# yamatokataoka/reinforcement-learning-replications

Measured on NVIDIA H100. Metric: ppo_update_transitions_per_sec, higher is better.
Workload: dtype f32

## Files before the change

reinforcement-learning-replications_b200/csrc/mlp_tc3.cu:

```cuda
#include <cuda_fp16.h>

#include <cmath>

#include "common.cuh"
#include "policy_head.cuh"
#include "tc2_common.cuh"
#include "tc_common.cuh"
#include "tc3.cuh"

namespace b200rl {

constexpr int T3_ROWS = 128;
constexpr int T3_CHAIN_WARPS = 8;
constexpr int T3_THREADS = T3_CHAIN_WARPS * 32 + 256;
constexpr int T3_WARPS = T3_THREADS / 32;

constexpr uint32_t S3_XB = 0;
constexpr uint32_t S3_H1 = 2 * T2_ACT;
constexpr uint32_t S3_H2 = S3_H1 + 2 * T2_ACT;
constexpr uint32_t S3_DZ2 = S3_H2 + 2 * T2_ACT;
constexpr uint32_t S3_DZ1 = S3_DZ2 + 2 * T2_ACT;
constexpr uint32_t T3_W1T = 32 * 128, T3_W2 = 64 * 128, T3_W3 = 16 * 128;
constexpr uint32_t S3_DO = S3_DZ1 + 2 * T2_ACT;
constexpr uint32_t S3_W = S3_DO + T2_ACT;
constexpr uint32_t S3_WNET = 2 * T3_W1T + 2 * T3_W2 + 2 * T3_W3;
constexpr uint32_t S3_OPERANDS_END = S3_W + S3_WNET;
constexpr uint32_t S3_BIAS = S3_OPERANDS_END;
constexpr uint32_t S3_DIST = S3_BIAS + 2 * 640;
constexpr uint32_t S3_SCALE = S3_DIST + 256;
constexpr uint32_t S3_XS = S3_SCALE + 128;
constexpr uint32_t S3_RED = S3_XS + 256;
constexpr uint32_t S3_BARS = S3_RED + 4 * 8 * T3_WARPS;
constexpr uint32_t S3_TOTAL = S3_BARS + 128;
constexpr uint32_t T3_SMEM_BYTES = S3_TOTAL + 1024;
static_assert(T3_SMEM_BYTES <= 227 * 1024, "mlp_tc3 shared memory");
constexpr uint32_t S3_END_DB3 = 0;
constexpr uint32_t S3_END_SC = 1024;

constexpr uint32_t ACC_GRAD_NET = 176;
constexpr uint32_t ACC_DB3 = 2 * ACC_GRAD_NET;
static_assert(ACC_DB3 + 4 * 16 <= ACC_COLS, "mlp_tc3 accumulator columns");
constexpr uint32_t ACC_DW2 = 0, ACC_DB2 = 64, ACC_DW1 = 80, ACC_DW3 = 144;

__device__ __forceinline__ uint32_t grad_acc_off(uint32_t pcol, int n, int row, int col) {
  const int rr = row & 63;
  const int t = 32 * (rr >> 4) + 4 * (rr & 7) + ((col >> 1) & 3);
  const int e = 2 * ((rr >> 3) & 1) + (col & 1);
  return pcol * ACC_LANES + (uint32_t)((row >> 6) * 64 * n + 4 * (128 * (col >> 3) + t) + e);
}

#ifdef B200RL_TC3_TIMING
__device__ unsigned long long g_tc3_t[64];
#endif

enum { C3_G = 0, C3_U1, C3_U2, C3_U3, C3_UH2, C3_UH1, C3_W1, C3_W2, C3_W3, C3_OW3, C3_OW2, C3_OW1, C3_OB, C3_N };

__device__ __forceinline__ void mbar_arrive_expect_tx(uint32_t bar, uint32_t bytes) {
  asm volatile("mbarrier.arrive.expect_tx.shared::cta.b64 _, [%0], %1;" ::"r"(bar), "r"(bytes) : "memory");
}
__device__ __forceinline__ void bulk_copy_g2s(uint32_t dst_smem, const void* src, uint32_t bytes, uint32_t bar) {
  asm volatile("cp.async.bulk.shared::cluster.global.mbarrier::complete_tx::bytes [%0], [%1], %2, [%3];" ::"r"(dst_smem),
               "l"(src), "r"(bytes), "r"(bar)
               : "memory");
}

__global__ void __launch_bounds__(128) pack_obs_kernel(const float* __restrict__ obs, long long n_rows, int n_in,
                                                       const float* __restrict__ absmax, uint8_t* __restrict__ ximg,
                                                       float* __restrict__ xscale, float* __restrict__ bad_flag) {
  __shared__ float s_xs[32];
  const int r = threadIdx.x;
  bool bad = false;
  if (r < 32) {
    const int e = r < n_in ? fit_exp(__ldg(absmax + r), bad) : 0;
    s_xs[r] = pow2i(e);
    if (blockIdx.x == 0) {
      xscale[r] = pow2i(e);
      xscale[32 + r] = pow2i(-e);
    }
  }
  __syncthreads();
  const long long tiles = (n_rows + T3_ROWS - 1) / T3_ROWS;
  for (long long t = blockIdx.x; t < tiles; t += gridDim.x) {
    const long long row = t * T3_ROWS + r;
    float x[32];
#pragma unroll
    for (int c = 0; c < 32; ++c) x[c] = 0.f;
    if (row < n_rows) {
      const float* src = obs + row * n_in;
      float rmax = 0.f, probe = 0.f;
#pragma unroll
      for (int c = 0; c < 31; ++c)
        if (c < n_in) {
          x[c] = __ldg(src + c) * s_xs[c];
          rmax = fmaxf(rmax, fabsf(x[c]));
          probe += x[c];
        }
      if (!(rmax <= T2_RANGE) || probe != probe) bad = true;
      if (rmax > 0.f && rmax < 0.03125f) bad = true;
      x[31] = 1.0f;
    }
    uint4 h[4], l[4];
#pragma unroll
    for (int j = 0; j < 4; ++j) {
      split2h(x[8 * j + 0], x[8 * j + 1], h[j].x, l[j].x);
      split2h(x[8 * j + 2], x[8 * j + 3], h[j].y, l[j].y);
      split2h(x[8 * j + 4], x[8 * j + 5], h[j].z, l[j].z);
      split2h(x[8 * j + 6], x[8 * j + 7], h[j].w, l[j].w);
    }
    uint8_t* dst = ximg + (size_t)t * T2_ACT + (size_t)r * 128;
#pragma unroll
    for (int j = 0; j < 4; ++j) {
      *reinterpret_cast<uint4*>(dst + ((j ^ (r & 7)) << 4)) = h[j];
      *reinterpret_cast<uint4*>(dst + (((4 + j) ^ (r & 7)) << 4)) = l[j];
    }
  }
  if (bad) *bad_flag = 1.0f;
}

template <int N, int TA, int TB, int TERMS, int KSTEPS>
__device__ __forceinline__ void wg_mma(float (&d)[N / 2], const uint32_t (&alo)[TERMS], const uint32_t (&blo)[TERMS],
                                       uint32_t a_hi, uint32_t b_hi, uint32_t a_k, uint32_t b_k, uint32_t accumulate) {
  wgmma_fence();
#pragma unroll
  for (int s = 0; s < TERMS; ++s)
#pragma unroll
    for (int k = 0; k < KSTEPS; ++k)
      wgmma_run<N, TA, TB>(d, ((uint64_t)a_hi << 32) | (alo[s] + (uint32_t)k * a_k),
                           ((uint64_t)b_hi << 32) | (blo[s] + (uint32_t)k * b_k), s == 0 && k == 0 ? accumulate : 1u);
  wgmma_commit();
  wgmma_wait_all();
}
template <int N, int TB, int KSTEPS>
__device__ __forceinline__ void chain_mma(float (&d)[N / 2], const Op2 a, const Op2 b) {
  const uint32_t alo[3] = {a.lo, a.lo + a.split_step, a.lo}, blo[3] = {b.lo + b.split_step, b.lo, b.lo};
#pragma unroll
  for (int i = 0; i < N / 2; ++i) d[i] = 0.f;
  wg_mma<N, K_MAJOR, TB, 3, KSTEPS>(d, alo, blo, a.hi, b.hi, a.k_step, b.k_step, 0u);
}
__device__ __forceinline__ float* grad_frag(float* acc_cta, uint32_t pcol) {
  const int t = (int)(threadIdx.x & 127u);
  return acc_cta + grad_acc_off(pcol, 0, 16 * (t >> 5) + ((t & 31) >> 2), 2 * (t & 3));
}
template <int N, int KSTEPS, int TERMS>
__device__ __forceinline__ void grad_products(float (&d)[N / 2], uint32_t a_lo, const Op2 a, const Op2 b, bool first) {
  uint32_t b_lo = b.lo;
  asm volatile("" : "+r"(a_lo), "+r"(b_lo));
#pragma unroll
  for (int s = 0; s < TERMS; ++s)
#pragma unroll
    for (int k = 0; k < KSTEPS; ++k)
      wgmma_run<N, MN_MAJOR, MN_MAJOR>(d, ((uint64_t)a.hi << 32) | (a_lo + (uint32_t)k * a.k_step),
                                       ((uint64_t)b.hi << 32) | (b_lo + (s + 1 < TERMS ? b.split_step : 0u) +
                                                                 (uint32_t)k * b.k_step),
                                       s == 0 && k == 0 ? (first ? 0u : 1u) : 1u);
}
template <int N>
__device__ __forceinline__ void grad_store(float* acc_cta, uint32_t pcol, int h, const float (&d)[N / 2]) {
  float* const frag = grad_frag(acc_cta, pcol) + 64 * N * h;
#pragma unroll
  for (int j = 0; j < N / 8; ++j)
    *reinterpret_cast<float4*>(frag + 512 * j) = make_float4(d[4 * j], d[4 * j + 1], d[4 * j + 2], d[4 * j + 3]);
}

__global__ void __launch_bounds__(T3_THREADS, 1) mlp_tc3_kernel(const Tc3Args p) {
  extern __shared__ uint8_t smem_raw[];
  const bool two = p.run_policy != 0 && p.run_value != 0;
  const int G = two ? (int)(gridDim.x >> 1) : (int)gridDim.x;
  const int c = two ? (int)blockIdx.x / G : (p.run_policy != 0 ? 0 : 1);
  const int slot = (int)blockIdx.x - c * (two ? G : 0);
  const bool run_p = p.run_policy != 0 && (p.stop_flag == nullptr || *p.stop_flag == 0);
  const bool run_v = p.run_value != 0;
  if (!(c == 0 ? run_p : run_v)) return;
  if (*p.x_bad != 0.f) return;
  const int tid = threadIdx.x, lane = tid & 31;
  float* const acc = p.acc_mem + (size_t)slot * ACC_CTA_FLOATS;
  const int warp = __shfl_sync(0xffffffffu, tid >> 5, 0);
  const uint32_t raw = smem_u32(smem_raw);
  const uint32_t base = (raw + 1023u) & ~1023u;
  uint8_t* sm = smem_raw + (base - raw);
  float* s_bias = reinterpret_cast<float*>(sm + S3_BIAS);
  float* s_dist = reinterpret_cast<float*>(sm + S3_DIST);
  float* s_scale = reinterpret_cast<float*>(sm + S3_SCALE);
  float* s_xs = reinterpret_cast<float*>(sm + S3_XS);
  float* s_red = reinterpret_cast<float*>(sm + S3_RED);
  int* s_bad = reinterpret_cast<int*>(sm + S3_BARS + 120);
  const uint32_t bars = base + S3_BARS;
  const int n_in = p.n_in;
  bool bad = false;
#ifdef B200RL_TC3_TIMING
  unsigned long long tacc[64];
  for (int i = 0; i < 64; ++i) tacc[i] = 0;
  const long long t_kernel0 = clock64();
#endif

  for (uint32_t i = S3_W / 16 + tid; i < S3_OPERANDS_END / 16; i += T3_THREADS) reinterpret_cast<uint4*>(sm)[i] = make_uint4(0, 0, 0, 0);
  if (tid == 0) *s_bad = 0;
  if (tid < 64) s_xs[tid] = __ldg(p.xscale + tid);
  float* s_par = reinterpret_cast<float*>(sm + S3_H1);
  static_assert(S3_W - S3_H1 >= 4 * (2 * 6000 + 64), "parameter staging area");
#pragma unroll 1
  for (int net = 0; net < 2; ++net) {
    const float* par = p.params[net];
    float* dst = s_par + (net == 0 ? 0 : p.P[0]);
#pragma unroll 8
    for (int i = tid; i < p.P[net]; i += T3_THREADS) dst[i] = (*(par + i));
  }
  __syncthreads();
#pragma unroll 1
  for (int net = 0; net < 2; ++net) {
    const Tc3Net& nn = p.net[net];
    const float* par = s_par + (net == 0 ? 0 : p.P[0]);
    float m1 = 0.f, m2 = 0.f, m3 = 0.f;
    for (int idx = tid; idx < nn.h1 * n_in; idx += T3_THREADS) {
      const float w = (*(par + nn.w_off[0] + idx)) * s_xs[32 + idx % n_in];
      m1 = fmaxf(m1, fabsf(w));
      if (w != w) bad = true;
    }
    for (int idx = tid; idx < nn.h2 * nn.h1; idx += T3_THREADS) {
      const float w = (*(par + nn.w_off[1] + idx));
      m2 = fmaxf(m2, fabsf(w));
      if (w != w) bad = true;
    }
    for (int idx = tid; idx < nn.n_out * nn.h2; idx += T3_THREADS) {
      const float w = (*(par + nn.w_off[2] + idx));
      m3 = fmaxf(m3, fabsf(w));
      if (w != w) bad = true;
    }
#pragma unroll
    for (int o = 16; o > 0; o >>= 1) {
      m1 = fmaxf(m1, __shfl_xor_sync(0xffffffffu, m1, o));
      m2 = fmaxf(m2, __shfl_xor_sync(0xffffffffu, m2, o));
      m3 = fmaxf(m3, __shfl_xor_sync(0xffffffffu, m3, o));
    }
    if (lane == 0) {
      s_red[warp * 8 + 4 * net + 0] = m1;
      s_red[warp * 8 + 4 * net + 1] = m2;
      s_red[warp * 8 + 4 * net + 2] = m3;
    }
  }
  __syncthreads();
  if (bad) *s_bad = 1;
  bad = false;
  if (tid < 2) {
    const int net = tid;
    const Tc3Net& nn = p.net[net];
    float m1 = 0.f, m2 = 0.f, m3 = 0.f;
    for (int w = 0; w < T3_WARPS; ++w) {
      m1 = fmaxf(m1, s_red[w * 8 + 4 * net + 0]);
      m2 = fmaxf(m2, s_red[w * 8 + 4 * net + 1]);
      m3 = fmaxf(m3, s_red[w * 8 + 4 * net + 2]);
    }
    bool b0 = false;
    const int ew1 = fit_exp(m1, b0), ew2 = fit_exp(m2, b0), ew3 = fit_exp(m3, b0);
    float typ;
    if (net == 1) {
      const float tm = __ldg(p.target_absmax);
      typ = (tm > 0.f && tm < INFINITY) ? 0.25f * tm : 1.f;
    } else if (p.dist == B200RL_DIST_GAUSSIAN) {
      float smin = INFINITY;
      for (int a = 0; a < nn.n_out; ++a) smin = fminf(smin, expf(__ldg(p.log_std + a)));
      typ = (smin > 0.f && smin < INFINITY) ? 1.f / smin : 1.f;
    } else {
      typ = 0.5f;
    }
    int eg = 3 + ilogbf(p.n_glob_f) - ilogbf(typ);
    eg = eg < -100 ? -100 : (eg > 100 ? 100 : eg);
    float* sc = s_scale + 16 * net;
    sc[C3_G] = pow2i(eg);
    sc[C3_U1] = pow2i(-ew1);
    sc[C3_U2] = pow2i(-(T2_H_EXP + ew2));
    sc[C3_U3] = pow2i(-(T2_H_EXP + ew3));
    sc[C3_UH2] = pow2i(-ew3);
    sc[C3_UH1] = pow2i(-ew2);
    sc[C3_W1] = pow2i(ew1);
    sc[C3_W2] = pow2i(ew2);
    sc[C3_W3] = pow2i(ew3);
    sc[C3_OW3] = pow2i(-(T2_H_EXP + eg));
    sc[C3_OW2] = pow2i(-(T2_H_EXP + eg));
    sc[C3_OW1] = pow2i(-eg);
    sc[C3_OB] = pow2i(-eg);
    if (b0) *s_bad = 1;
  }
  __syncthreads();
#pragma unroll 1
  for (int net = 0; net < 2; ++net) {
    const Tc3Net& nn = p.net[net];
    const float* par = s_par + (net == 0 ? 0 : p.P[0]);
    const uint32_t wb = S3_W;
    auto put = [&](uint32_t buf, uint32_t stride, int r, int c, float x) {
      const __half hb = __float2half_rn(x);
      const __half lb = __float2half_rn(x - __half2float(hb));
      const uint32_t off = buf + (uint32_t)r * 128u + ((uint32_t)((c >> 3) ^ (r & 7)) << 4) + ((uint32_t)(c & 7) << 1);
      *reinterpret_cast<__half*>(sm + off) = hb;
      *reinterpret_cast<__half*>(sm + off + stride) = lb;
    };
    const float* sc = s_scale + 16 * net;
    const float sw1 = sc[C3_W1], sw2 = sc[C3_W2], sw3 = sc[C3_W3];
    if (net == c) {
      for (int idx = tid; idx < nn.h1 * n_in; idx += T3_THREADS)
        put(wb, T3_W1T, idx % n_in, idx / n_in, ((*(par + nn.w_off[0] + idx)) * s_xs[32 + idx % n_in]) * sw1);
      for (int idx = tid; idx < nn.h2 * nn.h1; idx += T3_THREADS)
        put(wb + 2 * T3_W1T, T3_W2, idx / nn.h1, idx % nn.h1, (*(par + nn.w_off[1] + idx)) * sw2);
      for (int idx = tid; idx < nn.n_out * nn.h2; idx += T3_THREADS)
        put(wb + 2 * T3_W1T + 2 * T3_W2, T3_W3, idx / nn.h2, idx % nn.h2, (*(par + nn.w_off[2] + idx)) * sw3);
    }
    float* bb = s_bias + 160 * net;
    for (int i = tid; i < 64; i += T3_THREADS) {
      bb[i] = i < nn.h1 ? (*(par + nn.b_off[0] + i)) : 0.f;
      bb[64 + i] = i < nn.h2 ? (*(par + nn.b_off[1] + i)) : 0.f;
      if (!(fabsf(bb[i]) < INFINITY) || !(fabsf(bb[64 + i]) < INFINITY)) bad = true;
    }
    for (int i = tid; i < 16; i += T3_THREADS) {
      bb[128 + i] = i < nn.n_out ? (*(par + nn.b_off[2] + i)) : 0.f;
      if (!(fabsf(bb[128 + i]) < INFINITY)) bad = true;
    }
  }
  if (p.dist == B200RL_DIST_GAUSSIAN)
    for (int a = tid; a < p.net[0].n_out; a += T3_THREADS) {
      const NormalConsts nc = normal_consts(p.log_std, a);
      s_dist[a] = nc.var;
      s_dist[16 + a] = nc.log_scale;
      s_dist[32 + a] = nc.inv_2var;
      s_dist[48 + a] = nc.inv_var;
    }
  if (bad) *s_bad = 1;
  bad = false;
  if (tid == 0) {
    mbar_init(bars + 0, 1);
    mbar_init(bars + 8, 1);
    for (int i = 0; i < 3; ++i) {
      mbar_init(bars + 16 + 8 * i, 2);
      mbar_init(bars + 40 + 8 * i, 2);
    }
    fence_mbar_init();
  }
  fence_proxy_async_smem();
  __syncthreads();

  const long long num_tiles = (p.n_rows + T3_ROWS - 1) / T3_ROWS;
  const int cta_tiles = (int)((num_tiles - slot + G - 1) / G);

  constexpr int K = K_MAJOR, MN = MN_MAJOR;
  const uint32_t ub = base;
  auto bar_ready = [&](int s) { return bars + 16u + 8u * (uint32_t)(s - 3); };
  auto bar_done = [&](int s) { return bars + 40u + 8u * (uint32_t)(s - 3); };
  double sc[5] = {0, 0, 0, 0, 0};
  int rows_done = 0;
#ifdef B200RL_TC3_TIMING
  long long t_loop0 = 0, t_loop_end = 0;
#endif

  if (warp >= T3_CHAIN_WARPS) {
    const Op2 X_M = op2_mnmajor(ub + S3_XB, T2_ACT, 64);
    const Op2 X_M16 = op2_mnmajor(ub + S3_XB + 32, T2_ACT, 64);
    const Op2 DO_M = op2_at(op2_mnmajor(ub + S3_DO, T2_ACT, 32), c * 64);
    const Op2 H1_M = op2_mnmajor(ub + S3_H1, T2_ACT, T2_ACT), H2_M = op2_mnmajor(ub + S3_H2, T2_ACT, T2_ACT);
    const Op2 DZ2_M = op2_mnmajor(ub + S3_DZ2, T2_ACT, T2_ACT), DZ1_M = op2_mnmajor(ub + S3_DZ1, T2_ACT, T2_ACT);
    const int g = (warp - T3_CHAIN_WARPS) >> 2;
    const bool producer = g == 0;
    const uint32_t ah = (uint32_t)g * (T2_ACT >> 4);
    const uint32_t gcol = c * ACC_GRAD_NET;
    float w3[16], w2[32], b2[8], w1[32];
    auto load_x = [&](int k) {
      const uint32_t b = (uint32_t)(k & 1);
      const long long tile = slot + (long long)k * G;
      uint32_t e;
      asm volatile("{\n\t.reg .pred q;\n\telect.sync _|q, 0xffffffff;\n\tselp.u32 %0, 1, 0, q;\n\t}" : "=r"(e));
      if (e && (warp & 3) == 0) {
        mbar_arrive_expect_tx(bars + 8 * b, T2_ACT);
        bulk_copy_g2s(ub + S3_XB + b * T2_ACT, p.ximg + (size_t)tile * T2_ACT, T2_ACT, bars + 8 * b);
      }
      __syncwarp();
    };
    auto release = [&](int stage) {
      wgmma_commit();
      wgmma_wait_all();
      asm volatile("bar.sync %0, 128;" ::"r"(8 + g) : "memory");
      if ((tid & 127) == 0) mbar_arrive(bar_done(stage));
    };
    if (producer && cta_tiles > 0) load_x(0);
#pragma unroll 1
    for (int k = 0; k < cta_tiles; ++k) {
      const uint32_t xo = (uint32_t)(k & 1) * T2_ACT;
      const bool first = k == 0;
      if (producer && k + 1 < cta_tiles) {
        if (k > 0) mbar_wait(bar_done(5), (uint32_t)((k - 1) & 1));
        load_x(k + 1);
      }
#ifdef B200RL_TC3_TIMING
      long long it0 = clock64(), it1;
#define TC3_GSPLIT(s)                                                   \
  it1 = clock64();                                                      \
  tacc[40 + 3 * g + (s) - 3] += (unsigned long long)(it1 - it0);
#define TC3_GEND(s)                                                     \
  it0 = clock64();                                                      \
  tacc[46 + 3 * g + (s) - 3] += (unsigned long long)(it0 - it1);
#else
#define TC3_GSPLIT(s)
#define TC3_GEND(s)
#endif
      mbar_wait(bar_ready(3), (uint32_t)(k & 1));
      TC3_GSPLIT(3)
      wgmma_fence();
      grad_products<32, 8, 1>(w3, H2_M.lo + ah, H2_M, DO_M, first);
      release(3);
      TC3_GEND(3)
      mbar_wait(bar_ready(4), (uint32_t)(k & 1));
      TC3_GSPLIT(4)
      wgmma_fence();
      grad_products<64, 8, 2>(w2, DZ2_M.lo + ah, DZ2_M, H1_M, first);
      grad_products<16, 8, 1>(b2, DZ2_M.lo + ah, DZ2_M, op2_at(X_M16, xo), first);
      release(4);
      TC3_GEND(4)
      mbar_wait(bar_ready(5), (uint32_t)(k & 1));
      TC3_GSPLIT(5)
      wgmma_fence();
      grad_products<64, 8, 1>(w1, DZ1_M.lo + ah, DZ1_M, op2_at(X_M, xo), first);
      release(5);
      TC3_GEND(5)
#undef TC3_GSPLIT
#undef TC3_GEND
    }
    if (cta_tiles > 0) {
      grad_store<32>(acc, gcol + ACC_DW3, g, w3);
      grad_store<64>(acc, gcol + ACC_DW2, g, w2);
      grad_store<16>(acc, gcol + ACC_DB2, g, b2);
      grad_store<64>(acc, gcol + ACC_DW1, g, w1);
    }
#ifdef B200RL_TC3_TIMING
    if ((tid & 127) == 0 && blockIdx.x == 0) {
      for (int s = 0; s < 3; ++s) {
        g_tc3_t[40 + 3 * g + s] = tacc[40 + 3 * g + s];
        g_tc3_t[46 + 3 * g + s] = tacc[46 + 3 * g + s];
      }
      if (producer) g_tc3_t[52] = (unsigned long long)cta_tiles;
    }
#endif
  } else {
    const int wg = warp >> 2;
    const int quad = lane >> 2, q = lane & 3;
    const int r0 = 64 * wg + 16 * (warp & 3) + quad;
    const uint32_t rows = (uint32_t)wg * (64u * 128u);
    const Op2 X_K = op2_at(op2_kmajor(ub + S3_XB, 64), rows);
    const Op2 DO_K = op2_at(op2_kmajor(ub + S3_DO, 32), rows + c * 64);
    const Op2 H1_K = op2_at(op2_kmajor(ub + S3_H1, T2_ACT), rows), H2_K = op2_at(op2_kmajor(ub + S3_H2, T2_ACT), rows);
    const Op2 DZ2_K = op2_at(op2_kmajor(ub + S3_DZ2, T2_ACT), rows);
    const Op2 W1T_M = op2_mnmajor(ub + S3_W, 32 * 128, T3_W1T);
    const Op2 W2_K = op2_kmajor(ub + S3_W + 2 * T3_W1T, T3_W2), W2_M = op2_mnmajor(ub + S3_W + 2 * T3_W1T, 64 * 128, T3_W2);
    const Op2 W3_K = op2_kmajor(ub + S3_W + 2 * T3_W1T + 2 * T3_W2, T3_W3),
              W3_M = op2_mnmajor(ub + S3_W + 2 * T3_W1T + 2 * T3_W2, 16 * 128, T3_W3);
    const float* scl = s_scale + 16 * c;
    const float* bias = s_bias + 160 * c;
    const float sH = pow2i(T2_H_EXP), hh = pow2i(-2 * T2_H_EXP);
    const int A_out = p.net[0].n_out;

    auto frag_off = [&](uint32_t buf, int j, int r) -> uint32_t {
      return buf + (uint32_t)(r0 + 8 * r) * 128u + ((uint32_t)(j ^ quad) << 4) + 4u * (uint32_t)q;
    };
    auto store_pairs = [&](uint32_t buf, const float (&x)[32]) {
#pragma unroll
      for (int j = 0; j < 8; ++j)
#pragma unroll
        for (int r = 0; r < 2; ++r) {
          uint32_t h, l;
          split2h(x[4 * j + 2 * r], x[4 * j + 2 * r + 1], h, l);
          const uint32_t off = frag_off(buf, j, r);
          *reinterpret_cast<uint32_t*>(sm + off) = h;
          *reinterpret_cast<uint32_t*>(sm + off + T2_ACT) = l;
        }
    };
    auto act = [&](float (&z)[32], float unscale, const float* bs) {
#pragma unroll
      for (int g = 0; g < 2; ++g) {
        float t[16];
#pragma unroll
        for (int i = 0; i < 16; ++i) {
          const int e = 16 * g + i;
          t[i] = fmaf(z[e], unscale, bs[8 * (e >> 2) + 2 * q + (e & 1)]);
        }
        tanh16_scaled(t, sH);
#pragma unroll
        for (int i = 0; i < 16; ++i) z[16 * g + i] = t[i];
      }
    };
    auto dtanh = [&](float (&g)[32], float unscale, uint32_t buf) {
      const float one28 = 268435456.f;
      float m = 0.f;
#pragma unroll
      for (int j = 0; j < 8; ++j)
#pragma unroll
        for (int r = 0; r < 2; ++r) {
          const uint32_t off = frag_off(buf, j, r);
          const uint32_t hw = *reinterpret_cast<const uint32_t*>(sm + off);
          const uint32_t lw = *reinterpret_cast<const uint32_t*>(sm + off + T2_ACT);
          const float2 a = __half22float2(*reinterpret_cast<const __half2*>(&hw));
          const float2 b = __half22float2(*reinterpret_cast<const __half2*>(&lw));
          const float x0 = a.x + b.x, x1 = a.y + b.y;
          float& g0 = g[4 * j + 2 * r];
          float& g1 = g[4 * j + 2 * r + 1];
          g0 = (g0 * unscale) * fmaf(-x0, x0, one28);
          g1 = (g1 * unscale) * fmaf(-x1, x1, one28);
          m = fmaxf(m, fmaxf(fabsf(g0), fabsf(g1)));
        }
      if (!(m <= T2_RANGE)) bad = true;
    };
    auto wg_sync = [&]() {
      fence_proxy_async_smem();
      asm volatile("bar.sync %0, 128;" ::"r"(1 + wg) : "memory");
    };
    auto deliver = [&](int s) {
      wg_sync();
      if ((tid & 127) == 0) mbar_arrive(bar_ready(s));
    };
#ifdef B200RL_TC3_TIMING
    long long t_mark = 0;
#endif
    auto wait = [&](int s, uint32_t bar, uint32_t parity) {
#ifdef B200RL_TC3_TIMING
      const long long w0 = clock64();
#endif
      mbar_wait(bar, parity);
#ifdef B200RL_TC3_TIMING
      tacc[10 * wg + s - 1] += (unsigned long long)(clock64() - w0);
#endif
    };
    auto stage_end = [&](int s) {
#ifdef B200RL_TC3_TIMING
      const long long t = clock64();
      tacc[10 * wg + 4 + s] += (unsigned long long)(t - t_mark);
      t_mark = t;
#endif
    };

#ifdef B200RL_TC3_TIMING
    t_loop0 = clock64();
    t_mark = t_loop0;
#endif
    {
#pragma unroll 1
      for (int k = 0; k < cta_tiles; ++k) {
        const long long tile = slot + (long long)k * G;
        const uint32_t xo = (uint32_t)(k & 1) * T2_ACT;
        float d[32];
        wait(1, bars + 8 * (uint32_t)(k & 1), (uint32_t)((k >> 1) & 1));
        chain_mma<64, MN, 2>(d, op2_at(X_K, xo), W1T_M);
        act(d, scl[C3_U1], bias);
        if (k > 0) wait(1, bar_done(4), (uint32_t)((k - 1) & 1));
        store_pairs(S3_H1, d);
        wg_sync();
        stage_end(1);
        chain_mma<64, K, 4>(d, H1_K, W2_K);
        act(d, scl[C3_U2], bias + 64);
        store_pairs(S3_H2, d);
        wg_sync();
        stage_end(2);
        const int orow = r0 + 8 * q;
        const long long row = tile * T3_ROWS + orow;
        const bool owner = q < 2, valid = owner && row < p.n_rows;
        float pf_act[15], pf_in = 0.f, pf_old = 0.f;
#pragma unroll
        for (int a = 0; a < 15; ++a) pf_act[a] = 0.f;
        float* const s3p = acc + (ACC_DB3 + 16u * (uint32_t)((k + 2 * c) & 3)) * ACC_LANES + orow;
        if (valid) {
          if (c == 0) {
            if (p.dist == B200RL_DIST_GAUSSIAN) {
#pragma unroll
              for (int a = 0; a < 15; ++a)
                if (a < A_out) pf_act[a] = __ldg(p.actions + row * A_out + a);
            } else {
              pf_act[0] = __ldg(p.actions + row);
            }
            pf_in = __ldg(p.adv_raw + row);
            pf_old = __ldg(p.old_logp + row);
          } else {
            pf_in = __ldg(p.target + row);
          }
        }
        float o[8];
        chain_mma<16, K, 4>(o, H2_K, W3_K);
        float out[16];
#pragma unroll
        for (int j = 0; j < 2; ++j)
#pragma unroll
          for (int qq = 0; qq < 4; ++qq)
#pragma unroll
            for (int e = 0; e < 2; ++e) {
              const float v0 = __shfl_sync(0xffffffffu, o[4 * j + e], (lane & ~3) | qq);
              const float v1 = __shfl_sync(0xffffffffu, o[4 * j + 2 + e], (lane & ~3) | qq);
              out[8 * j + 2 * qq + e] = q == 0 ? v0 : v1;
            }
        float x0[8], x1[8];
#pragma unroll
        for (int j = 0; j < 8; ++j) x0[j] = x1[j] = 0.f;
        if (owner) {
          const float u3 = scl[C3_U3], sG = scl[C3_G];
          if (c == 0) {
            float dout[16];
#pragma unroll
            for (int a = 0; a < 16; ++a) {
              out[a] = fmaf(out[a], u3, bias[128 + a]);
              dout[a] = 0.f;
            }
            if (valid) {
              float lp, ent, dlp[16];
#pragma unroll
              for (int a = 0; a < 16; ++a) dlp[a] = 0.f;
              if (p.dist == B200RL_DIST_GAUSSIAN)
                gaussian_logp<15>(pf_act, out, s_dist + 16, VarRecip{s_dist + 48, s_dist + 32}, A_out, lp, ent, dlp);
              else
                categorical_logp<15>(out, (int)pf_act[0], A_out, lp, ent, dlp);
              float adv = pf_in;
              if (p.adv_stats != nullptr) {
                float adv_mean, adv_std;
                adv_mean_std(p.adv_stats, adv_mean, adv_std);
                adv = (adv - adv_mean) * (1.f / adv_std);
              }
              float coef;
              const float term = policy_loss(B200RL_LOSS_PPO_CLIP, lp, pf_old, adv, p.inv_n, p.clip_lo, p.clip_hi, coef);
#pragma unroll
              for (int a = 0; a < 15; ++a) dout[a] = coef * dlp[a];
              add_policy_row_sums(sc, term, lp, ent, pf_old, true);
            }
#pragma unroll
            for (int a = 0; a < 15; ++a) s3p[a * ACC_LANES] = (k >= 4 ? s3p[a * ACC_LANES] : 0.f) + dout[a];
#pragma unroll
            for (int j = 0; j < 8; ++j) {
              x0[j] = dout[j] * sG;
              x1[j] = j < 7 ? dout[8 + j] * sG : 0.f;
            }
          } else {
            float s3 = k >= 4 ? s3p[15 * ACC_LANES] : 0.f;
            if (valid) {
              float dout;
              sc[0] += (double)value_mse(fmaf(out[0], u3, bias[128]), pf_in, p.inv_n, dout);
              s3 += dout;
              x0[0] = dout * sG;
            }
            s3p[15 * ACC_LANES] = s3;
          }
          if (out_of_range8(x0) || out_of_range8(x1)) bad = true;
        }
        if (owner) {
          uint4 h0, l0, h1, l1;
          split2h(x0[0], x0[1], h0.x, l0.x);
          split2h(x0[2], x0[3], h0.y, l0.y);
          split2h(x0[4], x0[5], h0.z, l0.z);
          split2h(x0[6], x0[7], h0.w, l0.w);
          split2h(x1[0], x1[1], h1.x, l1.x);
          split2h(x1[2], x1[3], h1.y, l1.y);
          split2h(x1[4], x1[5], h1.z, l1.z);
          split2h(x1[6], x1[7], h1.w, l1.w);
          uint8_t* rowp = sm + S3_DO + (uint32_t)orow * 128u;
          const uint32_t sw = (uint32_t)(orow & 7), c4 = 4u * (uint32_t)c;
          *reinterpret_cast<uint4*>(rowp + (((c4 + 0u) ^ sw) << 4)) = h0;
          *reinterpret_cast<uint4*>(rowp + (((c4 + 1u) ^ sw) << 4)) = h1;
          *reinterpret_cast<uint4*>(rowp + (((c4 + 2u) ^ sw) << 4)) = l0;
          *reinterpret_cast<uint4*>(rowp + (((c4 + 3u) ^ sw) << 4)) = l1;
        }
        deliver(3);
        stage_end(3);
        chain_mma<64, MN, 1>(d, DO_K, W3_M);
        dtanh(d, scl[C3_UH2] * hh, S3_H2);
        store_pairs(S3_DZ2, d);
        deliver(4);
        stage_end(4);
        chain_mma<64, MN, 4>(d, DZ2_K, W2_M);
        dtanh(d, scl[C3_UH1] * hh, S3_H1);
        if (k > 0) wait(5, bar_done(5), (uint32_t)((k - 1) & 1));
        store_pairs(S3_DZ1, d);
        deliver(5);
        stage_end(5);
      }
    }
#ifdef B200RL_TC3_TIMING
    t_loop_end = clock64();
    if ((tid & 127) == 0 && blockIdx.x == 0)
      for (int i = 0; i < 10; ++i) g_tc3_t[10 * wg + i] = tacc[10 * wg + i];
#endif
    if (c == 0 && q < 2)
      for (int k = 0; k < cta_tiles; ++k) rows_done += (slot + (long long)k * G) * T3_ROWS + r0 + 8 * q < p.n_rows;
  }

  asm volatile("bar.sync 7, %0;" ::"n"(T3_THREADS) : "memory");
  {
    const int qw = warp & 3, part = warp >> 2;
    const int r = 32 * qw + lane;
    float* dst_row = p.partials + ((size_t)slot * 2 + (qw >> 1)) * (size_t)(p.P[0] + p.P[1]);
    const int m = 32 * (qw & 1) + lane;
    float v[16], w[16];
    const Tc3Net& nn = p.net[c];
    float* dst = dst_row + (c == 0 ? 0 : p.P[0]);
    const float* scn = s_scale + 16 * c;
    const bool have = cta_tiles > 0;
    const uint32_t gcol = c * ACC_GRAD_NET;
#pragma unroll 1
    for (int jb = part; jb < 8; jb += 4) {
      const uint32_t pcol = gcol + (jb < 4 ? ACC_DW2 : (jb < 6 ? ACC_DW1 : (jb == 6 ? ACC_DW3 : ACC_DB2)));
      const int pn = jb < 6 ? 64 : (jb == 6 ? 32 : 16);
      const int col = jb < 4 ? 16 * jb : (jb < 6 ? 16 * (jb - 4) : 0);
      const int col2 = jb < 4 ? col : (jb < 6 ? col + 32 : (jb == 6 ? 16 : col));
      if (have) {
#pragma unroll
        for (int j = 0; j < 16; ++j) {
          v[j] = acc[grad_acc_off(pcol, pn, r, col) + grad_acc_off(0, pn, 0, j)];
          w[j] = acc[grad_acc_off(pcol, pn, r, col2) + grad_acc_off(0, pn, 0, j)];
        }
      } else {
#pragma unroll
        for (int j = 0; j < 16; ++j) v[j] = w[j] = 0.f;
      }
      if (jb < 4) {
        const float u = scn[C3_OW2];
        if (m < nn.h2)
#pragma unroll
          for (int j = 0; j < 16; ++j)
            if (16 * jb + j < nn.h1) dst[nn.w_off[1] + m * nn.h1 + 16 * jb + j] = v[j] * u;
      } else if (jb < 6) {
        const int c0 = 16 * (jb - 4);
        const float u = scn[C3_OW1];
        if (m < nn.h1) {
#pragma unroll
          for (int j = 0; j < 16; ++j)
            if (c0 + j < n_in)
              dst[nn.w_off[0] + m * n_in + c0 + j] = ((v[j] + w[j]) * u) * s_xs[32 + c0 + j];
          if (jb == 5) dst[nn.b_off[0] + m] = (v[15] + w[15]) * scn[C3_OB];
        }
      } else if (jb == 6) {
        const float u = scn[C3_OW3];
        if (m < nn.h2)
#pragma unroll
          for (int a = 0; a < 15; ++a)
            if (a < nn.n_out) dst[nn.w_off[2] + a * nn.h2 + m] = (v[a] + w[a]) * u;
      } else {
        if (m < nn.h2) dst[nn.b_off[1] + m] = v[15] * scn[C3_OB];
      }
    }
  }
  float* e_db3 = reinterpret_cast<float*>(sm + S3_XB + S3_END_DB3);
  double* e_sc = reinterpret_cast<double*>(sm + S3_XB + S3_END_SC);
  {
    const int m = warp >> 2, rr = 32 * (warp & 3) + lane;
#pragma unroll
    for (int a = 0; a < 16; ++a) {
      const int cn = a == 15 ? 1 : 0;
      const bool have = cn == c && ((m - 2 * cn) & 3) < cta_tiles;
      float t = have ? acc[(ACC_DB3 + 16 * m + a) * ACC_LANES + rr] : 0.f;
#pragma unroll
      for (int o2 = 16; o2 > 0; o2 >>= 1) t += __shfl_xor_sync(0xffffffffu, t, o2);
      if (lane == 0) e_db3[warp * 16 + a] = t;
    }
  }
#pragma unroll
  for (int kk = 0; kk < 5; ++kk) {
    const double t = warp_sum(sc[kk]);
    if (lane == 0) e_sc[warp * 8 + kk] = t;
  }
  {
    const double t = warp_sum((double)rows_done);
    if (lane == 0) e_sc[warp * 8 + 5] = t;
  }
  __syncthreads();
  const size_t Ptot = (size_t)(p.P[0] + p.P[1]);
  if (tid < 16) {
    const int cn = tid == 15 ? 1 : 0, a = tid == 15 ? 0 : tid;
    if (cn == c && a < p.net[cn].n_out) {
      float t = 0.f;
      for (int w = 0; w < T3_WARPS; ++w) t += e_db3[w * 16 + tid];
      const size_t off = (cn == 0 ? 0 : (size_t)p.P[0]) + p.net[cn].b_off[2] + a;
      p.partials[((size_t)slot * 2) * Ptot + off] = t;
      p.partials[((size_t)slot * 2 + 1) * Ptot + off] = 0.f;
    }
  }
  const bool other_runs = c == 0 ? run_v : run_p;
  if (tid >= 32 && tid < 32 + 2 * B200RL_N_SCALARS && ((tid - 32) / B200RL_N_SCALARS == c || !other_runs)) {
    const int s = tid - 32;
    double t = 0.0;
    if (s / B200RL_N_SCALARS == c) {
      if (s < 6) {
        for (int w = 0; w < T3_CHAIN_WARPS; ++w) t += e_sc[w * 8 + s];
      } else if (s == 8) {
        for (int w = 0; w < T3_CHAIN_WARPS; ++w) t += e_sc[w * 8 + 0];
      }
    }
    p.scalar_partials[((size_t)slot * 2) * (2 * B200RL_N_SCALARS) + s] = t;
    p.scalar_partials[((size_t)slot * 2 + 1) * (2 * B200RL_N_SCALARS) + s] = 0.0;
  }
  if (bad) *s_bad = 1;
#ifdef B200RL_TC3_TIMING
  if (tid == 0 && blockIdx.x == 0) {
    g_tc3_t[53] = (unsigned long long)(t_loop0 - t_kernel0);
    g_tc3_t[54] = (unsigned long long)(t_loop_end - t_loop0);
    g_tc3_t[55] = (unsigned long long)(clock64() - t_loop_end);
  }
#endif

  __syncthreads();
  if (tid == 0 && *s_bad != 0) *p.status = 1.0f;
}

constexpr int RA3_WARPS = 8;

template <typename Acc>
__device__ __forceinline__ Acc ra3_gather(float* const* peers, int world, long long offset) {
  float x[RA3_MAX_WORLD];
#pragma unroll
  for (int r = 0; r < RA3_MAX_WORLD; ++r) {
    x[r] = 0.f;
    if (r < world) asm volatile("ld.relaxed.sys.global.f32 %0, [%1];" : "=f"(x[r]) : "l"(peers[r] + offset) : "memory");
  }
  Acc t = (Acc)0;
#pragma unroll
  for (int r = 0; r < RA3_MAX_WORLD; ++r)
    if (r < world) t += (Acc)x[r];
  return t;
}

__global__ void __launch_bounds__(RA3_WARPS * 32, 3) reduce_adam3_kernel(const Ra3Args a) {
  __shared__ float part[RA3_WARPS][32];
  __shared__ double spart[RA3_WARPS * 4][2 * B200RL_N_SCALARS];
  __shared__ double s_scal[2 * B200RL_N_SCALARS];
  const int lane = threadIdx.x & 31, warp = threadIdx.x >> 5;
  const long long Ptot = a.P[0] + a.P[1];
  const long long pidx = (long long)blockIdx.x * 32 + lane;
  const bool stopped_before = a.stop_flag != nullptr && *a.stop_flag != 0;
  const bool run_p = a.run_policy != 0 && !stopped_before, run_v = a.run_value != 0;
  const unsigned parity = a.seq & 1u;
  if (a.mode == 4) {
    if (threadIdx.x < 2 * B200RL_N_SCALARS)
      s_scal[threadIdx.x] = ra3_gather<double>(a.peers, a.world, parity * a.xchg_stride + Ptot + threadIdx.x);
  } else if (a.mode != 2) {
    const int k = lane & 15, cls = warp * 4 + (lane >> 4) * 2;
    for (int half = 0; half < 2; ++half) {
      double s = 0.0;
      for (int c = cls + half; c < a.rows; c += RA3_WARPS * 4) s += a.scalar_partials[(size_t)c * (2 * B200RL_N_SCALARS) + k];
      spart[cls + half][k] = s;
    }
    __syncthreads();
    if (threadIdx.x < 2 * B200RL_N_SCALARS) {
      double t = 0.0;
      for (int c = 0; c < RA3_WARPS * 4; ++c) t += spart[c][threadIdx.x];
      s_scal[threadIdx.x] = t;
    }
  } else {
    if (threadIdx.x < 2 * B200RL_N_SCALARS) s_scal[threadIdx.x] = (double)a.grad[Ptot + threadIdx.x];
  }
  __syncthreads();
  float g = 0.f;
  if (a.mode == 4) {
    if (warp == 0 && pidx < Ptot) {
      g = ra3_gather<float>(a.peers, a.world, parity * a.xchg_stride + pidx);
      if (a.grad != nullptr) a.grad[pidx] = g;
    }
  } else if (a.mode != 2) {
    float s0 = 0.f, s1 = 0.f, s2 = 0.f, s3 = 0.f;
    if (pidx < Ptot) {
      const float* qp = a.partials + pidx;
      int c = warp;
      for (; c + 3 * RA3_WARPS < a.rows; c += 4 * RA3_WARPS) {
        s0 += qp[(size_t)c * Ptot];
        s1 += qp[(size_t)(c + RA3_WARPS) * Ptot];
        s2 += qp[(size_t)(c + 2 * RA3_WARPS) * Ptot];
        s3 += qp[(size_t)(c + 3 * RA3_WARPS) * Ptot];
      }
      for (; c < a.rows; c += RA3_WARPS) s0 += qp[(size_t)c * Ptot];
    }
    part[warp][lane] = (s0 + s1) + (s2 + s3);
    __syncthreads();
    if (warp == 0 && pidx < Ptot) {
      g = part[0][lane];
#pragma unroll
      for (int w = 1; w < RA3_WARPS; ++w) g += part[w][lane];
      if (a.grad != nullptr) a.grad[pidx] = g;
    }
  } else if (warp == 0 && pidx < Ptot) {
    g = a.grad[pidx];
  }
  if (a.mode == 1) {
    if (blockIdx.x == 0 && threadIdx.x < 2 * B200RL_N_SCALARS) a.grad[Ptot + threadIdx.x] = (float)s_scal[threadIdx.x];
    return;
  }
  if (a.mode == 3 || a.mode == 5) {
    float* mine = a.peers[a.rank] + parity * a.xchg_stride;
    if (warp == 0 && pidx < Ptot) mine[pidx] = g;
    if (blockIdx.x == 0 && threadIdx.x < 2 * B200RL_N_SCALARS) mine[Ptot + threadIdx.x] = (float)s_scal[threadIdx.x];
    __threadfence();
    __syncthreads();
    if (threadIdx.x == 0) {
      const unsigned prev = atomicAdd(a.done_counter, 1u);
      if (prev == gridDim.x - 1) {
        *a.done_counter = 0u;
        __threadfence_system();
        unsigned* flag = reinterpret_cast<unsigned*>(a.peers[a.rank] + 2 * a.xchg_stride) + parity;
        asm volatile("st.release.sys.global.u32 [%0], %1;" ::"l"(flag), "r"(a.seq) : "memory");
      }
    }
    if (a.mode == 3) return;
    if (warp == 0 && lane < a.world) {
      const unsigned* flag = reinterpret_cast<const unsigned*>(a.peers[lane] + 2 * a.xchg_stride) + parity;
      const long long t0 = clock64();
      unsigned seen;
      for (;;) {
        asm volatile("ld.acquire.sys.global.u32 %0, [%1];" : "=r"(seen) : "l"(flag) : "memory");
        if (seen == a.seq) break;
        if (clock64() - t0 > 20000000000LL) {
          *a.comm_error = 1;
          break;
        }
        __nanosleep(64);
      }
    }
    __syncthreads();
    if (threadIdx.x < 2 * B200RL_N_SCALARS)
      s_scal[threadIdx.x] = ra3_gather<double>(a.peers, a.world, parity * a.xchg_stride + Ptot + threadIdx.x);
    if (warp == 0 && pidx < Ptot) {
      g = ra3_gather<float>(a.peers, a.world, parity * a.xchg_stride + pidx);
      if (a.grad != nullptr) a.grad[pidx] = g;
    }
    __syncthreads();
  }
  bool stop = !run_p;
  if (run_p && a.kl_limit_on) stop = (float)(s_scal[1] / a.n_global) > (float)a.kl_limit;
  if (warp == 0 && pidx < Ptot) {
    const int sidx = pidx < a.P[0] ? 0 : 1;
    const bool apply = sidx == 0 ? (run_p && !stop) : run_v;
    if (apply) {
      const Ra3Seg& sg = a.seg[sidx];
      const long long i = sidx == 0 ? pidx : pidx - a.P[0];
      float m = sg.m[i], v = sg.v[i];
      m = m + sg.one_minus_b1 * (g - m);
      v = v * sg.b2 + sg.one_minus_b2 * (g * g);
      const float denom = sqrtf(v) / sg.bc2_sqrt + sg.eps;
      sg.m[i] = m;
      sg.v[i] = v;
      sg.params[i] = sg.params[i] - sg.step_size * (m / denom);
    }
  }
  if (blockIdx.x == gridDim.x - 1 && threadIdx.x == 0) {
    if (run_p) {
      for (int k = 0; k < B200RL_N_SCALARS; ++k) a.slot_p[k] = s_scal[k];
      if (stop) *a.stop_flag = 1;
      else *a.applied_p += 1;
    }
    if (run_v) {
      for (int k = 0; k < B200RL_N_SCALARS; ++k) a.slot_v[k] = s_scal[B200RL_N_SCALARS + k];
      *a.applied_v += 1;
    }
  }
}

__global__ void __launch_bounds__(32) wait_peers_kernel(float* const* peers, int world, long long xchg_stride,
                                                        unsigned seq, int* comm_error) {
  if ((int)threadIdx.x >= world) return;
  const unsigned* flag = reinterpret_cast<const unsigned*>(peers[threadIdx.x] + 2 * xchg_stride) + (seq & 1u);
  const long long t0 = clock64();
  unsigned seen;
  do {
    asm volatile("ld.acquire.sys.global.u32 %0, [%1];" : "=r"(seen) : "l"(flag) : "memory");
    if (seen != seq && clock64() - t0 > 20000000000LL) {
      *comm_error = 1;
      break;
    }
  } while (seen != seq);
}

int launch_wait_peers(const Ra3Args& a, cudaStream_t s) {
  wait_peers_kernel<<<1, 32, 0, s>>>(a.peers, a.world, a.xchg_stride, a.seq, a.comm_error);
  B200RL_CUDA(cudaGetLastError());
  count_launch(1);
  return 0;
}

int tc3_configure() {
  static const int rc = []() -> int {
    return (int)cudaFuncSetAttribute(mlp_tc3_kernel, cudaFuncAttributeMaxDynamicSharedMemorySize, (int)T3_SMEM_BYTES);
  }();
  if (rc != 0) set_error("mlp_tc3: cudaFuncSetAttribute failed (%s)", cudaGetErrorString((cudaError_t)rc));
  return rc;
}

size_t tc3_ximg_bytes(int64_t n_rows) { return (size_t)((n_rows + T3_ROWS - 1) / T3_ROWS) * T2_ACT; }

bool tc3_shape_ok(const b200rl_mlp_desc& pol, const b200rl_mlp_desc& val) {
  auto ok = [](const b200rl_mlp_desc& d) {
    return d.n_layers == 3 && d.hidden_act == B200RL_ACT_TANH && d.out_act == B200RL_ACT_IDENTITY && d.sizes[0] >= 1 &&
           d.sizes[0] <= 31 && d.sizes[1] >= 1 && d.sizes[1] <= 64 && d.sizes[2] >= 1 && d.sizes[2] <= 64 &&
           d.sizes[3] >= 1 && d.sizes[3] <= 15;
  };
  return ok(pol) && ok(val) && pol.sizes[0] == val.sizes[0] && val.sizes[3] == 1;
}

int launch_pack_obs(const float* obs, int64_t n_rows, int n_in, const float* absmax, uint8_t* ximg, float* xscale,
                    float* bad_flag, cudaStream_t s) {
  const int64_t tiles = (n_rows + T3_ROWS - 1) / T3_ROWS;
  if (tiles <= 0) return 0;
  const int grid = (int)std::min<int64_t>(tiles, 8LL * 132);
  pack_obs_kernel<<<grid, 128, 0, s>>>(obs, n_rows, n_in, absmax, ximg, xscale, bad_flag);
  B200RL_CUDA(cudaGetLastError());
  count_launch(1);
  return 0;
}

int launch_mlp_tc3(const Tc3Args& k, cudaStream_t s) {
  if (tc3_configure()) return 1;
  const int grid = tc_grid(k.n_rows);
  B200RL_REQUIRE(grid > 0, "mlp_tc3: no CUDA device");
  Tc3Args kk = k;
  kk.acc_mem = acc_mem(grid, s);
  B200RL_REQUIRE(kk.acc_mem != nullptr, "mlp_tc3: no accumulator memory (allocation failed, or the stream is being captured): %s",
                 cudaGetErrorString(cudaGetLastError()));
  mlp_tc3_kernel<<<(k.run_policy && k.run_value) ? 2 * grid : grid, T3_THREADS, T3_SMEM_BYTES, s>>>(kk);
  B200RL_CUDA(cudaGetLastError());
  count_launch(1);
  return 0;
}

bool ra3_one_wave(long long p_total) {
  static const int per_sm = []() -> int {
    int n = 0;
    if (cudaOccupancyMaxActiveBlocksPerMultiprocessor(&n, reduce_adam3_kernel, RA3_WARPS * 32, 0) != cudaSuccess) {
      (void)cudaGetLastError();
      return 0;
    }
    return n;
  }();
  const int sms = device_sm_count();
  return sms > 0 && (p_total + 31) / 32 <= (long long)per_sm * sms;
}

int launch_reduce_adam3(const Ra3Args& a, cudaStream_t s) {
  const long long Ptot = a.P[0] + a.P[1];
  reduce_adam3_kernel<<<(int)((Ptot + 31) / 32), RA3_WARPS * 32, 0, s>>>(a);
  B200RL_CUDA(cudaGetLastError());
  count_launch(1);
  return 0;
}

}

#ifdef B200RL_TC3_TIMING
extern "C" int b200rl_debug_tc3_timing(unsigned long long* out64, int reset) {
  if (reset) {
    unsigned long long z[64] = {0};
    return (int)cudaMemcpyToSymbol(b200rl::g_tc3_t, z, sizeof(z));
  }
  return (int)cudaMemcpyFromSymbol(out64, b200rl::g_tc3_t, sizeof(unsigned long long) * 64);
}
#endif
```

Baseline: 13.22 million.

## Overlap ready-barrier arrival with chain wgmma and hoist per-row scalar loads

Splits the chain MMA into separate issue and wait steps, so a stage's ready barrier can be signalled to the gradient warps while the wgmma is still running. The per-row advantage mean and std are computed once per block and stored in the scale block, and the accumulator reads are hoisted ahead of the output MMA. The value net now shuffles only its single output column. Signalling ready before the MMA completes depends on the consumers reading only operands the in-flight wgmma does not overwrite, which adds ordering risk. Timing probes are also added behind a compile flag.

```diff
diff --git a/reinforcement-learning-replications_b200/csrc/mlp_tc3.cu b/reinforcement-learning-replications_b200/csrc/mlp_tc3.cu
--- a/reinforcement-learning-replications_b200/csrc/mlp_tc3.cu
+++ b/reinforcement-learning-replications_b200/csrc/mlp_tc3.cu
@@ -53,7 +53,9 @@
 __device__ unsigned long long g_tc3_t[64];
 #endif
 
-enum { C3_G = 0, C3_U1, C3_U2, C3_U3, C3_UH2, C3_UH1, C3_W1, C3_W2, C3_W3, C3_OW3, C3_OW2, C3_OW1, C3_OB, C3_N };
+enum { C3_G = 0, C3_U1, C3_U2, C3_U3, C3_UH2, C3_UH1, C3_W1, C3_W2, C3_W3, C3_OW3, C3_OW2, C3_OW1, C3_OB, C3_ADV_MEAN,
+       C3_ADV_RSTD, C3_N };
+static_assert(C3_N <= 16, "mlp_tc3 scale block");
 
 __device__ __forceinline__ void mbar_arrive_expect_tx(uint32_t bar, uint32_t bytes) {
   asm volatile("mbarrier.arrive.expect_tx.shared::cta.b64 _, [%0], %1;" ::"r"(bar), "r"(bytes) : "memory");
@@ -118,8 +120,9 @@
 }
 
 template <int N, int TA, int TB, int TERMS, int KSTEPS>
-__device__ __forceinline__ void wg_mma(float (&d)[N / 2], const uint32_t (&alo)[TERMS], const uint32_t (&blo)[TERMS],
-                                       uint32_t a_hi, uint32_t b_hi, uint32_t a_k, uint32_t b_k, uint32_t accumulate) {
+__device__ __forceinline__ void wg_mma_issue(float (&d)[N / 2], const uint32_t (&alo)[TERMS],
+                                             const uint32_t (&blo)[TERMS], uint32_t a_hi, uint32_t b_hi, uint32_t a_k,
+                                             uint32_t b_k, uint32_t accumulate) {
   wgmma_fence();
 #pragma unroll
   for (int s = 0; s < TERMS; ++s)
@@ -128,14 +131,22 @@
       wgmma_run<N, TA, TB>(d, ((uint64_t)a_hi << 32) | (alo[s] + (uint32_t)k * a_k),
                            ((uint64_t)b_hi << 32) | (blo[s] + (uint32_t)k * b_k), s == 0 && k == 0 ? accumulate : 1u);
   wgmma_commit();
+}
+template <int N, int TB, int KSTEPS>
+__device__ __forceinline__ void chain_mma_issue(float (&d)[N / 2], const Op2 a, const Op2 b) {
+  const uint32_t alo[3] = {a.lo, a.lo + a.split_step, a.lo}, blo[3] = {b.lo + b.split_step, b.lo, b.lo};
+#pragma unroll
+  for (int i = 0; i < N / 2; ++i) {
+    d[i] = 0.f;
+    asm volatile("" : "+f"(d[i])::"memory");
+  }
+  wg_mma_issue<N, K_MAJOR, TB, 3, KSTEPS>(d, alo, blo, a.hi, b.hi, a.k_step, b.k_step, 0u);
+}
+template <int N>
+__device__ __forceinline__ void chain_wait(float (&d)[N / 2]) {
   wgmma_wait_all();
-}
-template <int N, int TB, int KSTEPS>
-__device__ __forceinline__ void chain_mma(float (&d)[N / 2], const Op2 a, const Op2 b) {
-  const uint32_t alo[3] = {a.lo, a.lo + a.split_step, a.lo}, blo[3] = {b.lo + b.split_step, b.lo, b.lo};
-#pragma unroll
-  for (int i = 0; i < N / 2; ++i) d[i] = 0.f;
-  wg_mma<N, K_MAJOR, TB, 3, KSTEPS>(d, alo, blo, a.hi, b.hi, a.k_step, b.k_step, 0u);
+#pragma unroll
+  for (int i = 0; i < N / 2; ++i) asm volatile("" : "+f"(d[i])::"memory");
 }
 __device__ __forceinline__ float* grad_frag(float* acc_cta, uint32_t pcol) {
   const int t = (int)(threadIdx.x & 127u);
@@ -279,6 +290,12 @@
     sc[C3_OW2] = pow2i(-(T2_H_EXP + eg));
     sc[C3_OW1] = pow2i(-eg);
     sc[C3_OB] = pow2i(-eg);
+    if (net == 0 && p.adv_stats != nullptr) {
+      float adv_mean, adv_std;
+      adv_mean_std(p.adv_stats, adv_mean, adv_std);
+      sc[C3_ADV_MEAN] = adv_mean;
+      sc[C3_ADV_RSTD] = 1.f / adv_std;
+    }
     if (b0) *s_bad = 1;
   }
   __syncthreads();
@@ -508,8 +525,7 @@
       fence_proxy_async_smem();
       asm volatile("bar.sync %0, 128;" ::"r"(1 + wg) : "memory");
     };
-    auto deliver = [&](int s) {
-      wg_sync();
+    auto arrive_ready = [&](int s) {
       if ((tid & 127) == 0) mbar_arrive(bar_ready(s));
     };
 #ifdef B200RL_TC3_TIMING
@@ -529,6 +545,19 @@
       const long long t = clock64();
       tacc[10 * wg + 4 + s] += (unsigned long long)(t - t_mark);
       t_mark = t;
+#endif
+    };
+#ifdef B200RL_TC3_TIMING
+    long long t_prod = 0;
+#endif
+    auto product_begin = [&]() {
+#ifdef B200RL_TC3_TIMING
+      t_prod = clock64();
+#endif
+    };
+    auto product_end = [&](int s) {
+#ifdef B200RL_TC3_TIMING
+      tacc[20 + 10 * wg + s - 1] += (unsigned long long)(clock64() - t_prod);
 #endif
     };
 
@@ -543,13 +572,19 @@
         const uint32_t xo = (uint32_t)(k & 1) * T2_ACT;
         float d[32];
         wait(1, bars + 8 * (uint32_t)(k & 1), (uint32_t)((k >> 1) & 1));
-        chain_mma<64, MN, 2>(d, op2_at(X_K, xo), W1T_M);
+        product_begin();
+        chain_mma_issue<64, MN, 2>(d, op2_at(X_K, xo), W1T_M);
+        chain_wait<64>(d);
+        product_end(1);
         act(d, scl[C3_U1], bias);
         if (k > 0) wait(1, bar_done(4), (uint32_t)((k - 1) & 1));
         store_pairs(S3_H1, d);
         wg_sync();
         stage_end(1);
-        chain_mma<64, K, 4>(d, H1_K, W2_K);
+        product_begin();
+        chain_mma_issue<64, K, 4>(d, H1_K, W2_K);
+        chain_wait<64>(d);
+        product_end(2);
         act(d, scl[C3_U2], bias + 64);
         store_pairs(S3_H2, d);
         wg_sync();
@@ -576,19 +611,39 @@
             pf_in = __ldg(p.target + row);
           }
         }
+        float s3o[15];
+#pragma unroll
+        for (int a = 0; a < 15; ++a) s3o[a] = 0.f;
+        if (owner && k >= 4) {
+          if (c == 0) {
+#pragma unroll
+            for (int a = 0; a < 15; ++a) s3o[a] = s3p[a * ACC_LANES];
+          } else {
+            s3o[0] = s3p[15 * ACC_LANES];
+          }
+        }
         float o[8];
-        chain_mma<16, K, 4>(o, H2_K, W3_K);
+        product_begin();
+        chain_mma_issue<16, K, 4>(o, H2_K, W3_K);
+        chain_wait<16>(o);
+        product_end(3);
         float out[16];
-#pragma unroll
-        for (int j = 0; j < 2; ++j)
-#pragma unroll
-          for (int qq = 0; qq < 4; ++qq)
-#pragma unroll
-            for (int e = 0; e < 2; ++e) {
-              const float v0 = __shfl_sync(0xffffffffu, o[4 * j + e], (lane & ~3) | qq);
-              const float v1 = __shfl_sync(0xffffffffu, o[4 * j + 2 + e], (lane & ~3) | qq);
-              out[8 * j + 2 * qq + e] = q == 0 ? v0 : v1;
-            }
+        if (c == 0) {
+#pragma unroll
+          for (int j = 0; j < 2; ++j)
+#pragma unroll
+            for (int qq = 0; qq < 4; ++qq)
+#pragma unroll
+              for (int e = 0; e < 2; ++e) {
+                const float v0 = __shfl_sync(0xffffffffu, o[4 * j + e], (lane & ~3) | qq);
+                const float v1 = __shfl_sync(0xffffffffu, o[4 * j + 2 + e], (lane & ~3) | qq);
+                out[8 * j + 2 * qq + e] = q == 0 ? v0 : v1;
+              }
+        } else {
+          const float v0 = __shfl_sync(0xffffffffu, o[0], lane & ~3);
+          const float v1 = __shfl_sync(0xffffffffu, o[2], lane & ~3);
+          out[0] = q == 0 ? v0 : v1;
+        }
         float x0[8], x1[8];
 #pragma unroll
         for (int j = 0; j < 8; ++j) x0[j] = x1[j] = 0.f;
@@ -610,11 +665,7 @@
               else
                 categorical_logp<15>(out, (int)pf_act[0], A_out, lp, ent, dlp);
               float adv = pf_in;
-              if (p.adv_stats != nullptr) {
-                float adv_mean, adv_std;
-                adv_mean_std(p.adv_stats, adv_mean, adv_std);
-                adv = (adv - adv_mean) * (1.f / adv_std);
-              }
+              if (p.adv_stats != nullptr) adv = (adv - scl[C3_ADV_MEAN]) * scl[C3_ADV_RSTD];
               float coef;
               const float term = policy_loss(B200RL_LOSS_PPO_CLIP, lp, pf_old, adv, p.inv_n, p.clip_lo, p.clip_hi, coef);
 #pragma unroll
@@ -622,14 +673,14 @@
               add_policy_row_sums(sc, term, lp, ent, pf_old, true);
             }
 #pragma unroll
-            for (int a = 0; a < 15; ++a) s3p[a * ACC_LANES] = (k >= 4 ? s3p[a * ACC_LANES] : 0.f) + dout[a];
+            for (int a = 0; a < 15; ++a) s3p[a * ACC_LANES] = s3o[a] + dout[a];
 #pragma unroll
             for (int j = 0; j < 8; ++j) {
               x0[j] = dout[j] * sG;
               x1[j] = j < 7 ? dout[8 + j] * sG : 0.f;
             }
           } else {
-            float s3 = k >= 4 ? s3p[15 * ACC_LANES] : 0.f;
+            float s3 = s3o[0];
             if (valid) {
               float dout;
               sc[0] += (double)value_mse(fmaf(out[0], u3, bias[128]), pf_in, p.inv_n, dout);
@@ -657,25 +708,37 @@
           *reinterpret_cast<uint4*>(rowp + (((c4 + 2u) ^ sw) << 4)) = l0;
           *reinterpret_cast<uint4*>(rowp + (((c4 + 3u) ^ sw) << 4)) = l1;
         }
-        deliver(3);
+        wg_sync();
         stage_end(3);
-        chain_mma<64, MN, 1>(d, DO_K, W3_M);
+        product_begin();
+        chain_mma_issue<64, MN, 1>(d, DO_K, W3_M);
+        arrive_ready(3);
+        chain_wait<64>(d);
+        product_end(4);
         dtanh(d, scl[C3_UH2] * hh, S3_H2);
         store_pairs(S3_DZ2, d);
-        deliver(4);
+        wg_sync();
         stage_end(4);
-        chain_mma<64, MN, 4>(d, DZ2_K, W2_M);
+        product_begin();
+        chain_mma_issue<64, MN, 4>(d, DZ2_K, W2_M);
+        arrive_ready(4);
+        chain_wait<64>(d);
+        product_end(5);
         dtanh(d, scl[C3_UH1] * hh, S3_H1);
         if (k > 0) wait(5, bar_done(5), (uint32_t)((k - 1) & 1));
         store_pairs(S3_DZ1, d);
-        deliver(5);
+        wg_sync();
+        arrive_ready(5);
         stage_end(5);
       }
     }
 #ifdef B200RL_TC3_TIMING
     t_loop_end = clock64();
     if ((tid & 127) == 0 && blockIdx.x == 0)
-      for (int i = 0; i < 10; ++i) g_tc3_t[10 * wg + i] = tacc[10 * wg + i];
+      for (int i = 0; i < 10; ++i) {
+        g_tc3_t[10 * wg + i] = tacc[10 * wg + i];
+        g_tc3_t[20 + 10 * wg + i] = tacc[20 + 10 * wg + i];
+      }
 #endif
     if (c == 0 && q < 2)
       for (int k = 0; k < cta_tiles; ++k) rows_done += (slot + (long long)k * G) * T3_ROWS + r0 + 8 * q < p.n_rows;
```

Result: faster. 13.45 million, median of 6 (+1.7%).
